# OzAmram/CaloDiffusion

Hardware: AMD Instinct MI355X
Metric: sampled showers/sec (Dataset-2, 400-step DDIM) (higher is better)
Workload: dtype f32 (convs: fp32 operands as 2-term fp16 splits on the fp16 MFMA pipe, fp32 accumulate; attention/norms fp32)

## Files before the change

### calodiffusion_amd/csrc/conv_internal.h

```cpp
#pragma once
#include "kernels_conv.h"
#include "split16.h"
#include <cstdio>
#include <cstdlib>
#include <map>
#include <string>

namespace cd {

#define MFMA32(a, b, c) __builtin_amdgcn_mfma_f32_32x32x2f32((a), (b), (c), 0, 0, 0)
#define MFMA_BF16(a, b, c) __builtin_amdgcn_mfma_f32_32x32x16_bf16(__builtin_bit_cast(bf16x8, (a)), __builtin_bit_cast(bf16x8, (b)), (c), 0, 0, 0)

typedef __bf16 bf16x8 __attribute__((ext_vector_type(8)));
typedef __bf16 bf16x2 __attribute__((ext_vector_type(2)));

__device__ __forceinline__ unsigned pack_bf16(float lo, float hi) {
  const bf16x2 v = {(__bf16)lo, (__bf16)hi};
  return __builtin_bit_cast(unsigned, v);
}
__device__ __forceinline__ void split3(const f32x4 x, u32x2& t1, u32x2& t2, u32x2& t3) {
  f32x4 r = x;
  t1 = u32x2{pack_bf16(r[0], r[1]), pack_bf16(r[2], r[3])};
  r[0] -= __uint_as_float(t1[0] << 16); r[1] -= __uint_as_float(t1[0] & 0xffff0000u);
  r[2] -= __uint_as_float(t1[1] << 16); r[3] -= __uint_as_float(t1[1] & 0xffff0000u);
// ... 39 lines not shown
  int P;
  int cout, CTtot;
  int dbg;
  const float* coef;
  int act;
  float* ch_part;
  int* status = nullptr;
  GnDefer defer;
  int coef_lds_off = 0;
  const unsigned* in_absmax = nullptr;
  const float* add_src = nullptr;
};
bool try_launch_conv3_flat(const float* in0, int c0, const float* in1, int c1, const void* wpk, const float* bias, float* out,
                           int batch, int cout, const ConvGeom& g, hipStream_t s, const ConvFusion& fu,
                           int prec );
bool launch_conv_flat_split16(int VT, int CT, int NTERM, int geo, const ConvFlatArgs& a, dim3 grid, int threads, size_t lds, hipStream_t s);

std::map<std::string, int>& tune_cache();
template <typename F>
int autotune(const std::string& key, int ncand, F&& run, hipStream_t s) {
  auto it = tune_cache().find(key);
  if (it != tune_cache().end()) return it->second;
  hipStreamCaptureStatus st = hipStreamCaptureStatusNone;
  if (getenv("CD_NO_AUTOTUNE") || hipStreamIsCapturing(s, &st) != hipSuccess || st != hipStreamCaptureStatusNone || prof::enabled())
    return -1;
  hipEvent_t e0, e1;
  CD_HIP(hipEventCreate(&e0));
  CD_HIP(hipEventCreate(&e1));
  int best = 0;
  float best_ms = 1e30f;
  for (int i = 0; i < ncand; ++i) {
// ... 20 lines not shown
```

### calodiffusion_amd/csrc/kernels_conv_flat.hip

```cpp
#include "conv_internal.h"
#include "gn_defer.h"
#include <vector>

namespace cd {

template <int VT, int CT>
__global__ void __launch_bounds__(512, (VT * CT <= 2 ? 3 : 2)) conv3_flat_kernel(ConvFlatArgs a) {
  extern __shared__ __attribute__((aligned(16))) float lds[];
  const int tid = threadIdx.x, lane = tid & 63, wave = tid >> 6, nthreads = blockDim.x;
  const int b = blockIdx.y;
  const int ct0 = blockIdx.z * CT;
  const int HW = a.H * a.W;
  const int vox = a.D * HW;
  const int v0 = blockIdx.x * a.R;
  const int vend = min(v0 + a.R, vox);
  const int zA = v0 / HW - 1;
  const int zB = (vend - 1) / HW + 1;
  const int nstage = (zB - zA + 1) * HW;
  const int NZ = a.P * HW;
  const int half = lane >> 5, col = lane & 31;
  if (tid < 16) lds[NZ * 16 + tid] = 0.f;

  int nb[VT], rowm[VT], rowp[VT], ooff[VT];
  unsigned wmask[VT];
// ... 475 lines not shown
  const Dims3 d = g.in;
  const int CTtot = cout / 32;
  const int CTmax = CTtot <= 3 ? CTtot : 2;
  if (CTtot % CTmax) return false;
  const int HW = d.h * d.w, HWo = g.out.h * g.out.w;
  const size_t vox_bytes = prec == 3 ? 96 : (prec == 2 ? 80 : 64);
  auto planes = [&](int NT) { return ((32 * NT - 1) / HWo + 1) * g.sz + g.kd; };
  auto args_for = [&](int NT) {
    ConvFlatArgs a;
    a.in0 = in0; a.in1 = in1; a.c0 = c0; a.c1 = c1; a.wpk = (const float*)wpk; a.bias = bias; a.out = out;
    a.D = d.d; a.H = d.h; a.W = d.w; a.Do = g.out.d; a.Ho = g.out.h; a.Wo = g.out.w;
    a.R = 32 * NT; a.P = planes(NT); a.cout = cout; a.CTtot = CTtot;
    a.coef = fu.coef; a.act = fu.act; a.ch_part = fu.ch_part;
    return a;
  };
  auto launch = [&](int NT, int VT, int CT) -> bool {
    if (VT < 0) {
      const int NLW = -VT;
      ConvFlatArgs a = args_for(NT);
      a.dbg = 0;
      const size_t lds = 2 * ((size_t)a.P * HW + 1) * 96 + (size_t)NT * CT * 64 * 4;
      const int ups = (int)((g.out.vox() + a.R - 1) / a.R);
      const int total = ups * batch;
      const int nblk = total < 256 ? total : 256;
      dim3 grid((unsigned)nblk, 1, (unsigned)(CTtot / CT));
      if (fu.units) *fu.units = ups;
      const int threads = (NT + NLW) * 64;
      switch (CT) {
        case 1: launch_ws_inst<1>(a, grid, threads, lds, NLW, ups, total, s, geo); break;
        case 2: launch_ws_inst<2>(a, grid, threads, lds, NLW, ups, total, s, geo); break;
        case 3: launch_ws_inst<3>(a, grid, threads, lds, NLW, ups, total, s, geo); break;
        default: return false;
      }
      return true;
    }
    ConvFlatArgs a = args_for(NT);
    a.dbg = getenv("CD_FLAT_DBG") ? atoi(getenv("CD_FLAT_DBG")) : 0;
    a.status = fu.status; a.in_absmax = fu.in_absmax;
    a.add_src = prec >= 2 && !bias ? fu.add_src : nullptr;
    size_t lds = ((size_t)a.P * HW + 1) * vox_bytes;
    const size_t red = (size_t)(NT / VT) * CT * 32 * 2 * 4;
    if (lds < red) lds = red;
    if (fu.defer.part) {
      lds = (lds + 15) & ~(size_t)15;
      a.defer = fu.defer;
      a.coef_lds_off = (int)lds;
      lds += (size_t)fu.defer.C * 16 + gn_defer_scratch_bytes(fu.defer.C);
      if (lds > 160 * 1024) return false;
    }
    dim3 grid((unsigned)((g.out.vox() + a.R - 1) / a.R), (unsigned)batch, (unsigned)(CTtot / CT));
    if (fu.units) *fu.units = (int)grid.x;
    const int threads = (NT / VT) * 64;
    const bool launched = prec != 0 ? launch_conv_flat_split16(VT, CT, prec, geo, a, grid, threads, lds, s)
                                    : launch_conv_flat_f32(VT, CT, a, grid, threads, lds, s);
    if (!launched) return false;
    if (a.add_src && fu.add_done) *fu.add_done = 1;
    return true;
  };
  if (const char* ov = getenv("CD_FLAT_TILE")) {
    int nt, vt;
    if (sscanf(ov, "%d,%d", &nt, &vt) == 2 && nt % vt == 0 && nt / vt <= 8 && vt * CTmax <= 8 &&
        ((size_t)planes(nt) * HW + 1) * vox_bytes <= 160 * 1024 && (prec != 2 || vt * CTmax <= 4))
      return launch(nt, vt, CTmax);
  }
  static const int kCand[][2] = {{8, 2}, {4, 1}, {8, 1}, {12, 3}, {16, 2}, {16, 4}, {4, 2}, {6, 2}, {6, 3}, {2, 1},
                                 {3, 1}, {1, 1}, {2, 2}, {12, 2}, {8, 4}, {6, 1}, {3, 3}};
  struct Cand { int nt, vt, ct; };
  std::vector<Cand> cand;
  const bool small = g.out.vox() * batch <= 64 * 1024;
  for (int pass = 0; pass < (small && CTmax > 1 ? 2 : 1); ++pass) {
    const int CT = pass == 0 ? CTmax : 1;
    for (auto& c : kCand) {
      const int NT = c[0], VT = c[1];
      if (VT * CT > 8 || (CT == 3 && VT > 2)) continue;
      if (prec == 2 && VT * CT > 4) continue;
      static const bool no_extra_waves = getenv("CD_FLAT_NO_EXTRA_WAVES") != nullptr;
      const bool extra_ok = !no_extra_waves && g.out.vox() <= 128 && VT == 1 && NT <= 8;
      if ((int64_t)32 * (NT - 1) >= g.out.vox() && !extra_ok) continue;
      if (((size_t)planes(NT) * HW + 1) * vox_bytes > 150 * 1024) continue;
      if (pass == 1 && NT > 4) continue;
      cand.push_back({NT, VT, CT});
    }
  }
  if (prec == 3 && !getenv("CD_NO_WS")) {
    static const int kWs[][2] = {{8, 4}, {8, 2}, {4, 2}, {4, 4}, {8, 3}, {6, 2}, {2, 2}, {3, 1}, {1, 1}, {2, 1}};
    for (auto& c : kWs) {
      const int NMW = c[0], NLW = c[1];
      if ((int64_t)32 * (NMW - 1) >= g.out.vox()) continue;
      const size_t lds = 2 * ((size_t)planes(NMW) * HW + 1) * 96 + (size_t)NMW * CTmax * 64 * 4;
      if (lds > 160 * 1024 - 256) continue;
      cand.push_back({NMW, -NLW, CTmax});
    }
  }
  if (cand.empty()) return false;
  char key[192];
  std::snprintf(key, sizeof key, "flat%s g%d %dx%dx%d c%d+%d->%d b%d", prec == 3 ? "_bf16x3" : (prec == 2 ? "_f16x2" : "_f32"), geo,
                d.d, d.h, d.w, c0, c1, cout, batch);
  const int pick = autotune(key, (int)cand.size(), [&](int i) { launch(cand[i].nt, cand[i].vt, cand[i].ct); }, s);
  const Cand& c = cand[pick < 0 ? 0 : pick];
  return launch(c.nt, c.vt, c.ct);
}

}
```

### calodiffusion_amd/csrc/kernels_conv_flat16.hip

```cpp
#include "conv_internal.h"
#include "gn_defer.h"

namespace cd {

template <int VT, int CT, int KD, int KH, int KW, int SZ, int SXY, int NTERM>
__global__ void __launch_bounds__(512, (VT * CT * (NTERM == 2 ? 2 : 1) <= 2 ? 3 : 2)) conv3_flat_bf16x3_kernel(ConvFlatArgs a) {
  extern __shared__ __attribute__((aligned(16))) float lds[];
  char* ldsb = (char*)lds;
  constexpr int T = KD * KH * KW;
  constexpr int VB = NTERM == 3 ? 96 : 80;
  constexpr int WS = 64 * NTERM;
  const int tid = threadIdx.x, lane = tid & 63, wave = tid >> 6, nthreads = blockDim.x;
  const int b = blockIdx.y;
  const int ct0 = blockIdx.z * CT;
  const int HW = a.H * a.W;
  const int vox = a.D * HW;
  const int HWo = a.Ho * a.Wo;
  const int voxo = a.Do * HWo;
  const int v0 = blockIdx.x * a.R;
  const int vend = min(v0 + a.R, voxo);
  const float inv_hwo = 1.f / (float)HWo, inv_wo = 1.f / (float)a.Wo;
  auto fdiv = [](int x, float inv) { return (int)(((float)x + 0.5f) * inv); };
  const int zA = fdiv(v0, inv_hwo) * SZ - 1;
  const int zB = fdiv(vend - 1, inv_hwo) * SZ + KD - 2;
  const int nstage = (zB - zA + 1) * HW;
  const int NZ = a.P * HW;
  const int half = lane >> 5, col = lane & 31;
  if (a.defer.part) gn_defer_to_lds(a.defer, b, (float*)(ldsb + a.coef_lds_off), ldsb + a.coef_lds_off + a.defer.C * 16);
  const bool normed = a.coef || a.defer.part;
  if (tid < VB / 4) ((float*)(ldsb + (size_t)NZ * VB))[tid] = 0.f;

  int nb[VT], rowoff[VT][KH], ooff[VT];
  unsigned wmask[VT];
  bool any_valid = false;
#pragma unroll
  for (int vt = 0; vt < VT; ++vt) {
    const int v = v0 + (wave * VT + vt) * 32 + col;
    const bool valid = v < vend;
    const int vv = valid ? v : v0;
    const int oz = fdiv(vv, inv_hwo);
    const int r = vv - oz * HWo;
    const int oh = fdiv(r, inv_wo), ow = r - oh * a.Wo;
    const int ih0 = oh * SXY, iw0 = ow * SXY;
    nb[vt] = (oz * SZ - 1 - zA) * HW + ih0 * a.W + iw0;
    unsigned m = 0;
#pragma unroll
    for (int kh = 0; kh < KH; ++kh) {
      int ih = ih0 + kh - 1;
      ih = ih < 0 ? ih + a.H : (ih >= a.H ? ih - a.H : ih);
      ih = ih >= a.H ? ih - a.H : ih;
      rowoff[vt][kh] = (ih - ih0) * a.W;
    }
#pragma unroll
    for (int kw = 0; kw < KW; ++kw) {
      const int iw = iw0 + kw - 1;
      if (valid && iw >= 0 && iw < a.W) m |= 1u << kw;
    }
    wmask[vt] = m;
    ooff[vt] = valid ? v * a.cout : -1;
    any_valid |= valid;
  }
  const bool wave_active = __any(any_valid);

  f32x16 acc[VT][CT], accB[NTERM == 2 ? VT : 1][NTERM == 2 ? CT : 1];
#pragma unroll
  for (int vt = 0; vt < VT; ++vt)
#pragma unroll
    for (int ct = 0; ct < CT; ++ct)
#pragma unroll
      for (int r = 0; r < 16; ++r) {
        acc[vt][ct][r] = 0.f;
        if (NTERM == 2) accB[vt][ct][r] = 0.f;
      }

  float amax = 0.f;
  float gscale = 1.f, ginv = 1.f;
  if (NTERM == 2 && a.in_absmax) pow2_scale_for(*a.in_absmax, &gscale, &ginv);
  const int nsub = (a.c0 + a.c1) >> 4;
  const int gbase = zA * HW;
  const int nslots = nstage * 4;

  auto tap_voxel = [&](int vt, int tap) -> int {
#ifdef CD_FLAT_ABL_TAPS
    return nb[vt] + tap;
#endif
    const int kz = tap / (KH * KW), kh = (tap / KW) % KH, kw = tap % KW;
    const int n = nb[vt] + kz * HW + rowoff[vt][kh] + kw - 1;
    return ((wmask[vt] >> kw) & 1u) ? n : NZ;
  };

  for (int sc = 0; sc < nsub; ++sc) {
    const float* src;
    int ldc, coff;
    if (sc * 16 < a.c0) {
      src = a.in0; ldc = a.c0; coff = sc * 16;
    } else {
      src = a.in1; ldc = a.c1; coff = sc * 16 - a.c0;
    }
    const int pq = tid & 3;
    src += (size_t)b * vox * ldc + coff + pq * 4;
    f32x4 cf[4];
    if (a.defer.part) {
#pragma unroll
      for (int e = 0; e < 4; ++e) cf[e] = *(const f32x4*)(ldsb + a.coef_lds_off + (sc * 16 + pq * 4 + e) * 16);
    } else if (a.coef) {
#pragma unroll
      for (int e = 0; e < 4; ++e) cf[e] = *(const f32x4*)(a.coef + ((size_t)b * (a.c0 + a.c1) + sc * 16 + pq * 4 + e) * 4);
    }
    __syncthreads();
    for (int s0 = tid; s0 < ((a.dbg & 1) ? 0 : nslots); s0 += 4 * nthreads) {
      f32x4 val[4];
#pragma unroll
      for (int k = 0; k < 4; ++k) {
        const int sidx = s0 + k * nthreads;
        const int g = gbase + (sidx >> 2);
        val[k] = f32x4{0.f, 0.f, 0.f, 0.f};
        if (sidx < nslots && g >= 0 && g < vox) {
          val[k] = *(const f32x4*)(src + (size_t)g * ldc);
          if (normed) {
#pragma unroll
            for (int e = 0; e < 4; ++e) {
              float t = cf[e][0] * val[k][e] + cf[e][1];
              if (a.act) t = cd_fast_silu(t);
              val[k][e] = t + cf[e][2];
            }
          }
        }
      }
#pragma unroll
      for (int k = 0; k < 4; ++k) {
        const int sidx = s0 + k * nthreads;
        if (sidx < nslots) {
          char* d = ldsb + (size_t)(sidx >> 2) * VB + pq * 8;
          if (NTERM == 3) {
            u32x2 t1, t2, t3;
            split3(val[k], t1, t2, t3);
            *(u32x2*)d = t1;
            *(u32x2*)(d + 32) = t2;
            *(u32x2*)(d + 64) = t3;
          } else {
            const f32x4 vs = val[k] * gscale;
            amax = fmaxf(amax, fmaxf(fmaxf(fabsf(vs[0]), fabsf(vs[1])), fmaxf(fabsf(vs[2]), fabsf(vs[3]))));
            u32x2 t1, t2;
            split2(vs, t1, t2);
            *(u32x2*)d = t1;
            *(u32x2*)(d + 32) = t2;
          }
        }
      }
    }
    __syncthreads();
    if (!wave_active || (a.dbg & 2)) continue;

#pragma unroll
    for (int vt = 0; vt < VT; ++vt) asm volatile("" : "+v"(nb[vt]));

    const u32x4* wq = (const u32x4*)a.wpk + ((size_t)sc * T * a.CTtot + ct0) * WS + lane;
#ifndef CD_FLAT_WD
#define CD_FLAT_WD 3
#endif
#ifndef CD_FLAT_AD
#define CD_FLAT_AD 2
#endif
    constexpr bool DEEP = NTERM == 2;
    constexpr int WD = DEEP ? CD_FLAT_WD : 1, AD = DEEP ? CD_FLAT_AD : 1;
    u32x4 bw[WD + 1][CT][NTERM], av[AD + 1][VT][NTERM];
    auto load_w = [&](int tap) {
#pragma unroll
      for (int ct = 0; ct < CT; ++ct)
#pragma unroll
        for (int t = 0; t < NTERM; ++t) bw[tap % (WD + 1)][ct][t] = wq[((size_t)tap * a.CTtot + ct) * WS + t * 64];
    };
    auto load_a = [&](int tap) {
#pragma unroll
      for (int vt = 0; vt < VT; ++vt) {
        const char* p = ldsb + (size_t)tap_voxel(vt, tap) * VB + half * 16;
#pragma unroll
        for (int t = 0; t < NTERM; ++t) av[tap % (AD + 1)][vt][t] = *(const u32x4*)(p + t * 32);
      }
    };
#pragma unroll
    for (int t0 = 0; t0 < WD; ++t0) load_w(t0);
#pragma unroll
    for (int t0 = 0; t0 < AD; ++t0) load_a(t0);
#pragma unroll
    for (int tap = 0; tap < T; ++tap) {
      if (tap + WD < T) load_w(tap + WD);
      if (tap + AD < T) load_a(tap + AD);
      __builtin_amdgcn_sched_barrier(0);
      const int wc = tap % (WD + 1), ac = tap % (AD + 1);
#pragma unroll
// ... 6 lines not shown
            c = MFMA_BF16(av[ac][vt][1], bw[wc][ct][1], c);
            c = MFMA_BF16(av[ac][vt][0], bw[wc][ct][NTERM - 1], c);
            c = MFMA_BF16(av[ac][vt][1], bw[wc][ct][0], c);
            c = MFMA_BF16(av[ac][vt][0], bw[wc][ct][1], c);
            c = MFMA_BF16(av[ac][vt][0], bw[wc][ct][0], c);
            acc[vt][ct] = c;
          } else {
            acc[vt][ct] = MFMA_F16(av[ac][vt][0], bw[wc][ct][0], acc[vt][ct]);
            accB[vt][ct] = MFMA_F16(av[ac][vt][0], bw[wc][ct][1], accB[vt][ct]);
            accB[vt][ct] = MFMA_F16(av[ac][vt][1], bw[wc][ct][0], accB[vt][ct]);
          }
        }
    }
  }

  if (NTERM == 2) {
#pragma unroll
    for (int vt = 0; vt < VT; ++vt)
#pragma unroll
      for (int ct = 0; ct < CT; ++ct)
#pragma unroll
        for (int r = 0; r < 16; ++r) acc[vt][ct][r] = (acc[vt][ct][r] + accB[vt][ct][r] * (1.f / 2048.f)) * ginv;
  }
  if (NTERM == 2 && a.status && amax > 65504.f) atomicOr(a.status, 1);
  float* outb = a.out + (size_t)b * voxo * a.cout;
  float bv[CT];
#pragma unroll
  for (int ct = 0; ct < CT; ++ct) bv[ct] = a.bias ? a.bias[(ct0 + ct) * 32 + col] : 0.f;
  if (a.add_src) {
    const float* addb = a.add_src + (size_t)b * voxo * a.cout;
// ... 30 lines not shown
    for (int ct = 0; ct < CT; ++ct) s1[ct] = s2[ct] = 0.f;
#pragma unroll
    for (int vt = 0; vt < VT; ++vt)
#pragma unroll
      for (int r = 0; r < 16; ++r) {
        const int row = (r & 3) + 8 * (r >> 2) + 4 * half;
        const bool ok = __shfl(ooff[vt], row, 64) >= 0;
#pragma unroll
        for (int ct = 0; ct < CT; ++ct) {
          const float v = ok ? acc[vt][ct][r] + bv[ct] : 0.f;
          s1[ct] += v;
          s2[ct] += v * v;
        }
      }
    __syncthreads();
    const int nw = nthreads >> 6;
#pragma unroll
    for (int ct = 0; ct < CT; ++ct) {
      const float t1 = s1[ct] + __shfl_xor(s1[ct], 32, 64), t2 = s2[ct] + __shfl_xor(s2[ct], 32, 64);
      if (half == 0) {
        lds[((wave * CT + ct) * 32 + col) * 2] = t1;
        lds[((wave * CT + ct) * 32 + col) * 2 + 1] = t2;
      }
    }
    __syncthreads();
    for (int i = tid; i < CT * 32; i += nthreads) {
      float t1 = 0.f, t2 = 0.f;
      for (int w = 0; w < nw; ++w) {
        t1 += lds[((w * CT * 32) + i) * 2];
        t2 += lds[((w * CT * 32) + i) * 2 + 1];
      }
      float* dst = a.ch_part + (((size_t)b * gridDim.x + blockIdx.x) * a.cout + ct0 * 32 + i) * 2;
      dst[0] = t1;
      dst[1] = t2;
    }
  }
}

namespace {
template <int VT, int CT, int KD, int KH, int KW, int SZ, int SXY, int NTERM>
void launch_flat3_geo(const ConvFlatArgs& a, dim3 grid, int threads, size_t lds, hipStream_t s) {
  static bool attr_set = false;
  if (!attr_set) {
    CD_HIP(hipFuncSetAttribute((const void*)conv3_flat_bf16x3_kernel<VT, CT, KD, KH, KW, SZ, SXY, NTERM>,
                               hipFuncAttributeMaxDynamicSharedMemorySize, 160 * 1024));
    attr_set = true;
  }
  hipLaunchKernelGGL((conv3_flat_bf16x3_kernel<VT, CT, KD, KH, KW, SZ, SXY, NTERM>), grid, dim3(threads), lds, s, a);
  CD_HIP(hipGetLastError());
}
template <int VT, int CT, int NTERM>
void launch_flat3_inst(const ConvFlatArgs& a, dim3 grid, int threads, size_t lds, hipStream_t s, int geo = 0) {
  if (geo == 0) launch_flat3_geo<VT, CT, 3, 3, 3, 1, 1, NTERM>(a, grid, threads, lds, s);
  else if (geo == 1) launch_flat3_geo<VT, CT, 3, 4, 4, 2, 2, NTERM>(a, grid, threads, lds, s);
  else if (geo == 2) launch_flat3_geo<VT, CT, 3, 4, 4, 1, 2, NTERM>(a, grid, threads, lds, s);
  else launch_flat3_geo<VT, CT, 4, 4, 4, 2, 2, NTERM>(a, grid, threads, lds, s);
}
}

bool launch_conv_flat_split16(int VT, int CT, int NTERM, int geo, const ConvFlatArgs& a, dim3 grid, int threads, size_t lds, hipStream_t s) {
#define CD_FLAT_CASE(V, C)                                                                 \
  if (VT == V && CT == C) {                                                                \
    if (NTERM == 3) launch_flat3_inst<V, C, 3>(a, grid, threads, lds, s, geo);             \
    else if constexpr (V * C <= 4) launch_flat3_inst<V, C, 2>(a, grid, threads, lds, s, geo); \
    else return false;                                                                     \
    return true;                                                                           \
  }
  CD_FLAT_CASE(1, 1) CD_FLAT_CASE(2, 1) CD_FLAT_CASE(3, 1) CD_FLAT_CASE(4, 1)
  CD_FLAT_CASE(1, 2) CD_FLAT_CASE(2, 2) CD_FLAT_CASE(3, 2) CD_FLAT_CASE(4, 2)
  CD_FLAT_CASE(1, 3) CD_FLAT_CASE(2, 3)
#undef CD_FLAT_CASE
  return false;
}

}
```

### calodiffusion_amd/csrc/ops.hip

```cpp
#include "plan_internal.h"

namespace cd {

__global__ void to_cl_kernel(const float* __restrict__ src, float* __restrict__ dst, int channels, int64_t vox) {
  const int b = blockIdx.y;
  const int64_t total = vox * channels;
  for (int64_t i = (int64_t)blockIdx.x * 256 + threadIdx.x; i < total; i += (int64_t)gridDim.x * 256) {
    const int c = (int)(i % channels);
    const int64_t v = i / channels;
    dst[(size_t)b * total + i] = src[(size_t)b * total + (size_t)c * vox + v];
  }
}
__global__ void to_planar_kernel(const float* __restrict__ src, float* __restrict__ dst, int channels, int64_t vox) {
  const int b = blockIdx.y;
  const int64_t total = vox * channels;
  for (int64_t i = (int64_t)blockIdx.x * 256 + threadIdx.x; i < total; i += (int64_t)gridDim.x * 256) {
    const int64_t v = i % vox;
    const int c = (int)(i / vox);
    dst[(size_t)b * total + i] = src[(size_t)b * total + (size_t)v * channels + c];
  }
}
static void launch_transpose_to_cl(const float* ncdhw, float* ndhwc, int batch, int channels, int64_t vox, hipStream_t s) {
  int64_t bx = (vox * channels + 255) / 256;
  if (bx > 1024) bx = 1024;
// ... 66 lines not shown
    CD_REQUIRE(x && w && y && ch_part && units && scratch && chunks >= 0, "bad argument");
    CD_REQUIRE(cin % 32 == 0 && cout % 32 == 0, "channel counts must be multiples of 32");
    hipStream_t s = (hipStream_t)stream;
    launch_pack_weights_f16x2(w, scratch, cout, cin, 27, s);
    const Dims3 d{dims[0], dims[1], dims[2]};
    ConvGeom g{d, d, 3, 3, 3, 1, 1, 1};
    ConvFusion fu;
    int u = 0;
    fu.act = 1; fu.ch_part = ch_part; fu.units = &u; fu.zs_chunks = chunks;
    CD_REQUIRE(try_launch_conv_zslide(x, cin, nullptr, 0, scratch, bias, y, batch, cout, g, s, fu) && u > 0,
               "this grid is not eligible for the z-slide kernel");
    *units = u;
  });
}

int cd_op_cyl_conv_transpose(const float* x, const float* w, const float* bias, float* y, int batch, int channels,
                             const int32_t dims_in[3], int kernel_z, int stride_z, const int32_t out_pad[3],
                             void* scratch, void* stream) {
  return guarded([&] {
    CD_REQUIRE(x && w && y && scratch, "null argument");
    CD_REQUIRE(out_pad[0] == 0, "z output padding is always 0 (models.py:339)");
    hipStream_t s = (hipStream_t)stream;
    float* wpk = (float*)scratch;
    launch_pack_weights(w, wpk, channels, channels, kernel_z * 16, true, s);
    float* wpk16 = wpk + ((packed_weight_floats(channels, channels, kernel_z * 16) + 63) & ~(size_t)63);
    launch_pack_weights_f16x2(w, wpk16, channels, channels, kernel_z * 16, s, true, false);
    const Dims3 din{dims_in[0], dims_in[1], dims_in[2]};
    const Dims3 dout{(din.d - 1) * stride_z - 2 + kernel_z, 2 * din.h + out_pad[1], 2 * din.w + out_pad[2]};
    launch_conv_transpose_mfma(x, channels, wpk, bias, y, batch, channels, din, dout, kernel_z, stride_z, s, wpk16, nullptr);
  });
// ... 173 lines not shown
```

### calodiffusion_amd/engine.py

```python
from __future__ import annotations

import ctypes as C
import os
from typing import Dict, Optional, Sequence

import numpy as np
import torch

_HERE = os.path.dirname(os.path.abspath(__file__))
LIB_PATH = os.environ.get("CALODIFF_LIB") or os.path.join(_HERE, "lib", "libcalodiff_hip.so")

CD_MAX_SIZES = 8
CD_ABI_VERSION = 3
TIME_KINDS = {"log": 0, "sigma": 1, "raw": 2}
OBJECTIVES = {"hybrid": 0, "noise_pred": 1, "mean_pred": 2}
LOSS_TYPES = {"l2": 0, "l1": 1, "mse": 2, "huber": 3}


class CdUnetDesc(C.Structure):
    _fields_ = [
        ("struct_size", C.c_uint32),
        ("grid", C.c_int32 * 3),
        ("in_channels", C.c_int32),
        ("n_sizes", C.c_int32),
# ... 140 lines not shown
                                            C.c_uint64, C.c_uint64, _P, _P, _P, C.c_double, C.c_double, C.c_double, C.c_float, _P, _P,
                                            C.c_size_t, _P]),
    "cd_classifier_dropout_mask": (C.c_int, [C.c_uint64, C.c_uint64, C.c_int, C.c_float, C.c_int, C.c_int, _P, _P]),
    "cd_set_conv_precision": (C.c_int, [C.c_char_p]),
    "cd_get_conv_precision": (C.c_char_p, []),
    "cd_profile_begin": (C.c_int, []),
    "cd_profile_end": (C.c_int, [C.c_char_p, C.c_int]),
    "cd_loss_hybrid_l2": (C.c_int, [_P, C.c_int, _P, _P, _P, _P, _P, _P, C.c_size_t, _P]),
    "cd_loss_hybrid": (C.c_int, [_P, C.c_int, _P, _P, _P, _P, C.c_int, _P, _P, C.c_size_t, _P]),
    "cd_op_to_channels_last": (C.c_int, [_P, _P, C.c_int, C.c_int, C.c_int64, _P]),
    "cd_op_to_ncdhw": (C.c_int, [_P, _P, C.c_int, C.c_int, C.c_int64, _P]),
    "cd_op_cyl_conv": (C.c_int, [_P, C.c_int, _P, C.c_int, _P, _P, _P, C.c_int, C.c_int, C.POINTER(C.c_int32),
                                 C.POINTER(C.c_int32), C.POINTER(C.c_int32), _P, _P]),
    "cd_op_zslide_conv": (C.c_int, [_P, C.c_int, _P, _P, _P, _P, C.POINTER(C.c_int), C.c_int, C.c_int, C.POINTER(C.c_int32), C.c_int,
                                    _P, _P]),
    "cd_op_cyl_conv_transpose": (C.c_int, [_P, _P, _P, _P, C.c_int, C.c_int, C.POINTER(C.c_int32), C.c_int, C.c_int,
                                           C.POINTER(C.c_int32), _P, _P]),
    "cd_op_init_conv": (C.c_int, [_P, _P, _P, _P, C.c_int, C.c_int, C.c_int, C.POINTER(C.c_int32), _P, _P]),
    "cd_op_init_pair_conv": (C.c_int, [_P, _P, _P, _P, _P, C.c_int, _P, _P, _P, C.c_int, C.c_int, _P, _P, _P, C.POINTER(C.c_int), C.c_int,
                                       C.POINTER(C.c_int32), C.c_int, _P, _P]),
    "cd_op_group_norm": (C.c_int, [_P, _P, _P, _P, C.c_int, C.c_int, C.c_int64, C.c_int, C.c_int, _P, _P, _P, _P]),
    "cd_op_resnet_block": (C.c_int, [_P, C.c_int, _P, C.c_int, C.POINTER(_P), _P, _P, C.c_int, C.c_int,
                                     C.POINTER(C.c_int32), C.c_int, _P, C.c_size_t, _P]),
    "cd_op_linear_attention": (C.c_int, [_P, C.POINTER(_P), _P, C.c_int, C.c_int, C.POINTER(C.c_int32), _P, C.c_size_t, _P]),
    "cd_op_conv_backward": (C.c_int, [_P, C.c_int, _P, C.c_int, _P, _P, _P, _P, _P, C.c_int, C.c_int, C.POINTER(C.c_int32),
                                      C.POINTER(C.c_int32), C.POINTER(C.c_int32), _P, C.c_size_t, _P]),
    "cd_op_conv_transpose_backward": (C.c_int, [_P, _P, _P, _P, _P, _P, C.c_int, C.c_int, C.POINTER(C.c_int32), C.c_int, C.c_int,
                                                C.POINTER(C.c_int32), _P, C.c_size_t, _P]),
    "cd_op_group_norm_backward": (C.c_int, [_P, _P, _P, _P, _P, _P, _P, _P, C.c_int, C.c_int, C.c_int64, C.c_int, C.c_int, _P,
                                            C.c_size_t, _P]),
# ... 788 lines not shown

    def zslide_conv_chunked(self, x_cl, w, bias, chunks=0):
        x_cl, w = _dev32(x_cl, "x"), _dev32(w, "w")
        B, D, H, W, cin = x_cl.shape
        cout = w.shape[0]
        y = torch.empty((B, D, H, W, cout), dtype=torch.float32, device=x_cl.device)
        cap = (D * H * W + 31) // 32
        part = torch.zeros((B, cap, cout, 2), dtype=torch.float32, device=x_cl.device)
        units = C.c_int()
        sc = self.scratch(B, max(cin, cout), D * H * W)
        _check(self.lib.cd_op_zslide_conv(x_cl.data_ptr(), cin, w.data_ptr(), _ptr(bias), y.data_ptr(), part.data_ptr(), C.byref(units),
                                          B, cout, _i32x3((D, H, W)), int(chunks), sc.data_ptr(), _stream()))
        u = units.value
        return y, part.view(-1)[:B * u * cout * 2].view(B, u, cout, 2).double().sum(1)

    def cyl_conv_transpose(self, x_cl, w, bias, kernel_z, stride_z, out_pad):
        x_cl, w = _dev32(x_cl, "x"), _dev32(w, "w")
        B, D, H, W, c = x_cl.shape
        od = ((D - 1) * stride_z - 2 + kernel_z, 2 * H + out_pad[1], 2 * W + out_pad[2])
        y = torch.empty((B,) + od + (c,), dtype=torch.float32, device=x_cl.device)
        sc = self.scratch(B, c, int(np.prod(od)))
        _check(self.lib.cd_op_cyl_conv_transpose(x_cl.data_ptr(), w.data_ptr(), _ptr(bias), y.data_ptr(), B, c,
                                                 _i32x3((D, H, W)), kernel_z, stride_z, _i32x3(out_pad), sc.data_ptr(),
                                                 _stream()))
        return y

    def init_conv(self, x_ncdhw, w, bias):
        x, w = _dev32(x_ncdhw, "x"), _dev32(w, "w")
        B, cin, D, H, W = x.shape
        cout = w.shape[0]
# ... 106 lines not shown
```

### include/calodiff.h

```cpp
#ifndef CALODIFF_H
#define CALODIFF_H

#include <stddef.h>
#include <stdint.h>

#ifdef __cplusplus
extern "C" {
#endif

#define CD_OK 0
#define CD_EINVAL -1
#define CD_EHIP -2
#define CD_ENOGPU -3
#define CD_EWEIGHTS -4
#define CD_EWORKSPACE -5

#define CD_MAX_SIZES 8

#define CD_ABI_VERSION 3

#define CD_TIME_LOG 0
#define CD_TIME_SIGMA 1
#define CD_TIME_RAW 2

// ... 261 lines not shown
int cd_classifier_dropout_mask(uint64_t seed, uint64_t step, int layer, float dropout_p, int rows, int n, uint8_t* mask, void* stream);

int cd_set_conv_precision(const char* mode);
const char* cd_get_conv_precision(void);

int cd_profile_begin(void);
int cd_profile_end(char* json, int cap);

int cd_op_to_channels_last(const float* ncdhw, float* ndhwc, int batch, int channels, int64_t voxels, void* stream);
int cd_op_to_ncdhw(const float* ndhwc, float* ncdhw, int batch, int channels, int64_t voxels, void* stream);
int cd_op_cyl_conv(const float* x0, int c0, const float* x1, int c1, const float* w, const float* bias, float* y,
                   int batch, int cout, const int32_t dims_in[3], const int32_t kernel[3], const int32_t stride[3],
                   void* scratch, void* stream);
int cd_op_zslide_conv(const float* x, int cin, const float* w, const float* bias, float* y, float* ch_part, int* units, int batch,
                      int cout, const int32_t dims[3], int chunks, void* scratch, void* stream);
int cd_op_cyl_conv_transpose(const float* x, const float* w, const float* bias, float* y, int batch, int channels,
                             const int32_t dims_in[3], int kernel_z, int stride_z, const int32_t out_pad[3],
                             void* scratch, void* stream);
int cd_op_init_conv(const float* x_ncdhw, const float* w, const float* bias, float* y, int batch, int cin, int cout,
                    const int32_t dims[3], void* scratch, void* stream);
int cd_op_init_pair_conv(const float* x, const float* w0, const float* b0, const float* w1, const float* b1, int cin, const float* r_w,
                         const float* z_d, const float* phi_h, int use_rz, int use_phi, const float* scale_b, float* y, float* ch_part,
                         int* units, int batch, const int32_t dims[3], int slabs, void* scratch, void* stream);
int cd_op_group_norm(const float* x, float* y, const float* gamma, const float* beta, int batch, int channels,
                     int64_t voxels, int groups, int silu, const float* add_bc, const float* residual,
                     void* scratch, void* stream);
int cd_op_resnet_block(const float* x0, int c0, const float* x1, int c1, const float* const* w, const float* cond, float* y,
                       int batch, int cout, const int32_t dims[3], int groups, void* workspace, size_t workspace_bytes,
                       void* stream);
int cd_op_linear_attention(const float* x, const float* const* w, float* y, int batch, int channels, const int32_t dims[3],
// ... 22 lines not shown
```

Measured before the change: 97.17.

## Add flat-conv block forms covering all channel tiles and split-K channel groups

Adds two new launch forms for the f16x2 flat conv kernel. In the first, one block covers every output channel tile, so the staged input image is shared across channel tiles instead of being restaged per grid z-slice. In the second, for small grids, two wave groups each take half the input channel sub-blocks and reduce their partial accumulators through LDS. The change also precomputes per-row LDS tap offsets with edge masks, adds these forms to the autotune candidates, and exposes a test entry point. The cost is larger blocks (up to 1024 threads), extra LDS and extra synchronisation.

```diff
diff --git a/calodiffusion_amd/csrc/conv_internal.h b/calodiffusion_amd/csrc/conv_internal.h
--- a/calodiffusion_amd/csrc/conv_internal.h
+++ b/calodiffusion_amd/csrc/conv_internal.h
@@ -77,7 +77,8 @@
 bool try_launch_conv3_flat(const float* in0, int c0, const float* in1, int c1, const void* wpk, const float* bias, float* out,
                            int batch, int cout, const ConvGeom& g, hipStream_t s, const ConvFusion& fu,
                            int prec );
-bool launch_conv_flat_split16(int VT, int CT, int NTERM, int geo, const ConvFlatArgs& a, dim3 grid, int threads, size_t lds, hipStream_t s);
+bool launch_conv_flat_split16(int VT, int CT, int NTERM, int geo, const ConvFlatArgs& a, dim3 grid, int threads, size_t lds, hipStream_t s,
+                              int form = 0);
 
 std::map<std::string, int>& tune_cache();
 template <typename F>
diff --git a/calodiffusion_amd/csrc/kernels_conv_flat.hip b/calodiffusion_amd/csrc/kernels_conv_flat.hip
--- a/calodiffusion_amd/csrc/kernels_conv_flat.hip
+++ b/calodiffusion_amd/csrc/kernels_conv_flat.hip
@@ -513,7 +513,15 @@
     a.coef = fu.coef; a.act = fu.act; a.ch_part = fu.ch_part;
     return a;
   };
-  auto launch = [&](int NT, int VT, int CT) -> bool {
+  const int nsub = (c0 + c1) / 16;
+  auto form_ok = [&](int NT, int form) {
+    return prec == 2 && geo <= 2 && (form == 1 || (form == 2 && nsub >= 2)) && NT >= 1 && form * CTtot * NT <= 16;
+  };
+  auto lds_image = [&](int NT, int VT, int form) {
+    return (size_t)(prec == 2 && VT == 1 ? g.kw * 80 : 0) + (form == 2 ? 2 : 1) * ((size_t)planes(NT) * HW + 1) * vox_bytes;
+  };
+  auto launch = [&](int NT, int VT, int CT, int form = 0) -> bool {
+    if (form != 0 && !form_ok(NT, form)) return false;
     if (VT < 0) {
       const int NLW = -VT;
       ConvFlatArgs a = args_for(NT);
@@ -537,9 +545,11 @@
     a.dbg = getenv("CD_FLAT_DBG") ? atoi(getenv("CD_FLAT_DBG")) : 0;
     a.status = fu.status; a.in_absmax = fu.in_absmax;
     a.add_src = prec >= 2 && !bias ? fu.add_src : nullptr;
-    size_t lds = ((size_t)a.P * HW + 1) * vox_bytes;
-    const size_t red = (size_t)(NT / VT) * CT * 32 * 2 * 4;
+    size_t lds = lds_image(NT, VT, form);
+    size_t red = (size_t)(NT / VT) * CT * 32 * 2 * 4;
+    if (form != 0) red = (size_t)NT * CTtot * (form == 2 ? 32 * 64 * 4 : 32 * 2 * 4);
     if (lds < red) lds = red;
+    if (lds > 160 * 1024) return false;
     if (fu.defer.part) {
       lds = (lds + 15) & ~(size_t)15;
       a.defer = fu.defer;
@@ -547,24 +557,28 @@
       lds += (size_t)fu.defer.C * 16 + gn_defer_scratch_bytes(fu.defer.C);
       if (lds > 160 * 1024) return false;
     }
-    dim3 grid((unsigned)((g.out.vox() + a.R - 1) / a.R), (unsigned)batch, (unsigned)(CTtot / CT));
-    if (fu.units) *fu.units = (int)grid.x;
-    const int threads = (NT / VT) * 64;
-    const bool launched = prec != 0 ? launch_conv_flat_split16(VT, CT, prec, geo, a, grid, threads, lds, s)
+    dim3 grid((unsigned)((g.out.vox() + a.R - 1) / a.R), (unsigned)batch, (unsigned)(form != 0 ? 1 : CTtot / CT));
+    const int threads = form != 0 ? form * CTtot * NT * 64 : (NT / VT) * 64;
+    const bool launched = prec != 0 ? launch_conv_flat_split16(VT, CT, prec, geo, a, grid, threads, lds, s, form)
                                     : launch_conv_flat_f32(VT, CT, a, grid, threads, lds, s);
     if (!launched) return false;
+    if (fu.units) *fu.units = (int)grid.x;
     if (a.add_src && fu.add_done) *fu.add_done = 1;
     return true;
   };
   if (const char* ov = getenv("CD_FLAT_TILE")) {
-    int nt, vt;
-    if (sscanf(ov, "%d,%d", &nt, &vt) == 2 && nt % vt == 0 && nt / vt <= 8 && vt * CTmax <= 8 &&
-        ((size_t)planes(nt) * HW + 1) * vox_bytes <= 160 * 1024 && (prec != 2 || vt * CTmax <= 4))
+    int nt, vt, form = 0;
+    const int nf = sscanf(ov, "%d,%d,%d", &nt, &vt, &form);
+    if (nf == 3 && form != 0 && prec == 2) {
+      if (vt == 1 && form_ok(nt, form) && launch(nt, 1, 1, form)) return true;
+    } else if (nf >= 2 && nt % vt == 0 && nt / vt <= 8 && vt * CTmax <= 8 &&
+               ((size_t)planes(nt) * HW + 1) * vox_bytes <= 160 * 1024 && (prec != 2 || vt * CTmax <= 4)) {
       return launch(nt, vt, CTmax);
+    }
   }
   static const int kCand[][2] = {{8, 2}, {4, 1}, {8, 1}, {12, 3}, {16, 2}, {16, 4}, {4, 2}, {6, 2}, {6, 3}, {2, 1},
                                  {3, 1}, {1, 1}, {2, 2}, {12, 2}, {8, 4}, {6, 1}, {3, 3}};
-  struct Cand { int nt, vt, ct; };
+  struct Cand { int nt, vt, ct, form; };
   std::vector<Cand> cand;
   const bool small = g.out.vox() * batch <= 64 * 1024;
   for (int pass = 0; pass < (small && CTmax > 1 ? 2 : 1); ++pass) {
@@ -578,7 +592,25 @@
       if ((int64_t)32 * (NT - 1) >= g.out.vox() && !extra_ok) continue;
       if (((size_t)planes(NT) * HW + 1) * vox_bytes > 150 * 1024) continue;
       if (pass == 1 && NT > 4) continue;
-      cand.push_back({NT, VT, CT});
+      cand.push_back({NT, VT, CT, 0});
+    }
+  }
+  if (CTtot >= 2 && geo != 0) {
+    for (int NT : {2, 1, 4}) {
+      if (!form_ok(NT, 1) || NT * CTtot > 8 || (int64_t)32 * (NT - 1) >= g.out.vox() || lds_image(NT, 1, 1) > 150 * 1024) continue;
+      cand.push_back({NT, 1, 1, 1});
+    }
+  }
+  static const int n_simd = [] {
+    int dev = 0, cus = 0;
+    CD_HIP(hipGetDevice(&dev));
+    CD_HIP(hipDeviceGetAttribute(&cus, hipDeviceAttributeMultiprocessorCount, dev));
+    return 4 * cus;
+  }();
+  if ((g.out.vox() + 31) / 32 * batch * CTtot < 2 * (int64_t)n_simd) {
+    for (int NT : {1, 2}) {
+      if (!form_ok(NT, 2) || 2 * NT * CTtot > 8 || (int64_t)32 * (NT - 1) >= g.out.vox() || lds_image(NT, 1, 2) > 150 * 1024) continue;
+      cand.push_back({NT, 1, 1, 2});
     }
   }
   if (prec == 3 && !getenv("CD_NO_WS")) {
@@ -588,16 +620,16 @@
       if ((int64_t)32 * (NMW - 1) >= g.out.vox()) continue;
       const size_t lds = 2 * ((size_t)planes(NMW) * HW + 1) * 96 + (size_t)NMW * CTmax * 64 * 4;
       if (lds > 160 * 1024 - 256) continue;
-      cand.push_back({NMW, -NLW, CTmax});
+      cand.push_back({NMW, -NLW, CTmax, 0});
     }
   }
   if (cand.empty()) return false;
   char key[192];
   std::snprintf(key, sizeof key, "flat%s g%d %dx%dx%d c%d+%d->%d b%d", prec == 3 ? "_bf16x3" : (prec == 2 ? "_f16x2" : "_f32"), geo,
                 d.d, d.h, d.w, c0, c1, cout, batch);
-  const int pick = autotune(key, (int)cand.size(), [&](int i) { launch(cand[i].nt, cand[i].vt, cand[i].ct); }, s);
+  const int pick = autotune(key, (int)cand.size(), [&](int i) { launch(cand[i].nt, cand[i].vt, cand[i].ct, cand[i].form); }, s);
   const Cand& c = cand[pick < 0 ? 0 : pick];
-  return launch(c.nt, c.vt, c.ct);
-}
-
-}
+  return launch(c.nt, c.vt, c.ct, c.form);
+}
+
+}
diff --git a/calodiffusion_amd/csrc/kernels_conv_flat16.hip b/calodiffusion_amd/csrc/kernels_conv_flat16.hip
--- a/calodiffusion_amd/csrc/kernels_conv_flat16.hip
+++ b/calodiffusion_amd/csrc/kernels_conv_flat16.hip
@@ -3,16 +3,29 @@
 
 namespace cd {
 
-template <int VT, int CT, int KD, int KH, int KW, int SZ, int SXY, int NTERM>
-__global__ void __launch_bounds__(512, (VT * CT * (NTERM == 2 ? 2 : 1) <= 2 ? 3 : 2)) conv3_flat_bf16x3_kernel(ConvFlatArgs a) {
+template <int VT, int CT, int KD, int KH, int KW, int SZ, int SXY, int NTERM, int FORM = 0, int MAXT = 512>
+__global__ void __launch_bounds__(MAXT, (MAXT > 512 ? 4 : (VT * CT * (NTERM == 2 ? 2 : 1) <= 2 ? 3 : 2)))
+conv3_flat_bf16x3_kernel(ConvFlatArgs a) {
   extern __shared__ __attribute__((aligned(16))) float lds[];
   char* ldsb = (char*)lds;
   constexpr int T = KD * KH * KW;
   constexpr int VB = NTERM == 3 ? 96 : 80;
   constexpr int WS = 64 * NTERM;
+  constexpr bool PRE = NTERM == 2 && VT == 1;
+  constexpr int IMG = PRE ? KW * VB : 0;
+  constexpr int NG = FORM == 2 ? 2 : 1;
+  static_assert(FORM == 0 || (VT == 1 && CT == 1 && PRE), "forms 1 and 2: one (row tile, channel tile) pair per wave");
   const int tid = threadIdx.x, lane = tid & 63, wave = tid >> 6, nthreads = blockDim.x;
   const int b = blockIdx.y;
-  const int ct0 = blockIdx.z * CT;
+  const int ntile = a.R >> 5;
+  int ct0 = blockIdx.z * CT, tile0 = wave * VT, grp = 0;
+  if (FORM != 0) {
+    const int ws = __builtin_amdgcn_readfirstlane(wave);
+    const int q = (int)(((float)ws + 0.5f) * (1.f / (float)ntile));
+    tile0 = ws - q * ntile;
+    grp = q >= a.CTtot ? 1 : 0;
+    ct0 = q - grp * a.CTtot;
+  }
   const int HW = a.H * a.W;
   const int vox = a.D * HW;
   const int HWo = a.Ho * a.Wo;
@@ -28,14 +41,19 @@
   const int half = lane >> 5, col = lane & 31;
   if (a.defer.part) gn_defer_to_lds(a.defer, b, (float*)(ldsb + a.coef_lds_off), ldsb + a.coef_lds_off + a.defer.C * 16);
   const bool normed = a.coef || a.defer.part;
-  if (tid < VB / 4) ((float*)(ldsb + (size_t)NZ * VB))[tid] = 0.f;
+  const int img_bytes = (NZ + 1) * VB;
+  if (PRE) {
+    for (int i = tid; i < IMG / 4; i += nthreads) ((float*)ldsb)[i] = 0.f;
+  } else if (tid < VB / 4) {
+    ((float*)(ldsb + (size_t)NZ * VB))[tid] = 0.f;
+  }
 
   int nb[VT], rowoff[VT][KH], ooff[VT];
   unsigned wmask[VT];
   bool any_valid = false;
 #pragma unroll
   for (int vt = 0; vt < VT; ++vt) {
-    const int v = v0 + (wave * VT + vt) * 32 + col;
+    const int v = v0 + (tile0 + vt) * 32 + col;
     const bool valid = v < vend;
     const int vv = valid ? v : v0;
     const int oz = fdiv(vv, inv_hwo);
@@ -61,6 +79,16 @@
     any_valid |= valid;
   }
   const bool wave_active = __any(any_valid);
+  unsigned rb[PRE ? KD * KH : 1], mkL = 0, mkR = 0;
+  if constexpr (PRE) {
+#pragma unroll
+    for (int kz = 0; kz < KD; ++kz)
+#pragma unroll
+      for (int kh = 0; kh < KH; ++kh)
+        rb[kz * KH + kh] = (unsigned)(IMG + grp * img_bytes + (nb[0] + kz * HW + rowoff[0][kh] - 1) * VB + half * 16);
+    mkL = (wmask[0] & 1u) ? ~0u : 0u;
+    mkR = ((wmask[0] >> (KW - 1)) & 1u) ? ~0u : 0u;
+  }
 
   f32x16 acc[VT][CT], accB[NTERM == 2 ? VT : 1][NTERM == 2 ? CT : 1];
 #pragma unroll
@@ -89,71 +117,83 @@
     return ((wmask[vt] >> kw) & 1u) ? n : NZ;
   };
 
-  for (int sc = 0; sc < nsub; ++sc) {
-    const float* src;
-    int ldc, coff;
-    if (sc * 16 < a.c0) {
-      src = a.in0; ldc = a.c0; coff = sc * 16;
-    } else {
-      src = a.in1; ldc = a.c1; coff = sc * 16 - a.c0;
-    }
-    const int pq = tid & 3;
-    src += (size_t)b * vox * ldc + coff + pq * 4;
-    f32x4 cf[4];
-    if (a.defer.part) {
-#pragma unroll
-      for (int e = 0; e < 4; ++e) cf[e] = *(const f32x4*)(ldsb + a.coef_lds_off + (sc * 16 + pq * 4 + e) * 16);
-    } else if (a.coef) {
-#pragma unroll
-      for (int e = 0; e < 4; ++e) cf[e] = *(const f32x4*)(a.coef + ((size_t)b * (a.c0 + a.c1) + sc * 16 + pq * 4 + e) * 4);
-    }
-    __syncthreads();
-    for (int s0 = tid; s0 < ((a.dbg & 1) ? 0 : nslots); s0 += 4 * nthreads) {
-      f32x4 val[4];
-#pragma unroll
-      for (int k = 0; k < 4; ++k) {
-        const int sidx = s0 + k * nthreads;
-        const int g = gbase + (sidx >> 2);
-        val[k] = f32x4{0.f, 0.f, 0.f, 0.f};
-        if (sidx < nslots && g >= 0 && g < vox) {
-          val[k] = *(const f32x4*)(src + (size_t)g * ldc);
-          if (normed) {
-#pragma unroll
-            for (int e = 0; e < 4; ++e) {
-              float t = cf[e][0] * val[k][e] + cf[e][1];
-              if (a.act) t = cd_fast_silu(t);
-              val[k][e] = t + cf[e][2];
+  for (int sc0 = 0; sc0 < nsub; sc0 += NG) {
+#pragma unroll
+    for (int j = 0; j < NG; ++j) {
+      const int sc = sc0 + j;
+      if (j > 0 && sc >= nsub) break;
+      const float* src;
+      int ldc, coff;
+      if (sc * 16 < a.c0) {
+        src = a.in0; ldc = a.c0; coff = sc * 16;
+      } else {
+        src = a.in1; ldc = a.c1; coff = sc * 16 - a.c0;
+      }
+      const int pq = tid & 3;
+      src += (size_t)b * vox * ldc + coff + pq * 4;
+      f32x4 cf[4];
+      if (a.defer.part) {
+#pragma unroll
+        for (int e = 0; e < 4; ++e) cf[e] = *(const f32x4*)(ldsb + a.coef_lds_off + (sc * 16 + pq * 4 + e) * 16);
+      } else if (a.coef) {
+#pragma unroll
+        for (int e = 0; e < 4; ++e) cf[e] = *(const f32x4*)(a.coef + ((size_t)b * (a.c0 + a.c1) + sc * 16 + pq * 4 + e) * 4);
+      }
+      if (j == 0) __syncthreads();
+      char* img = ldsb + IMG + j * img_bytes;
+      for (int s0 = tid; s0 < ((a.dbg & 1) ? 0 : nslots); s0 += 4 * nthreads) {
+        f32x4 val[4];
+#pragma unroll
+        for (int k = 0; k < 4; ++k) {
+          const int sidx = s0 + k * nthreads;
+          const int g = gbase + (sidx >> 2);
+          val[k] = f32x4{0.f, 0.f, 0.f, 0.f};
+          if (sidx < nslots && g >= 0 && g < vox) {
+            val[k] = *(const f32x4*)(src + (size_t)g * ldc);
+            if (normed) {
+#pragma unroll
+              for (int e = 0; e < 4; ++e) {
+                float t = cf[e][0] * val[k][e] + cf[e][1];
+                if (a.act) t = cd_fast_silu(t);
+                val[k][e] = t + cf[e][2];
+              }
             }
           }
         }
-      }
-#pragma unroll
-      for (int k = 0; k < 4; ++k) {
-        const int sidx = s0 + k * nthreads;
-        if (sidx < nslots) {
-          char* d = ldsb + (size_t)(sidx >> 2) * VB + pq * 8;
-          if (NTERM == 3) {
-            u32x2 t1, t2, t3;
-            split3(val[k], t1, t2, t3);
-            *(u32x2*)d = t1;
-            *(u32x2*)(d + 32) = t2;
-            *(u32x2*)(d + 64) = t3;
-          } else {
-            const f32x4 vs = val[k] * gscale;
-            amax = fmaxf(amax, fmaxf(fmaxf(fabsf(vs[0]), fabsf(vs[1])), fmaxf(fabsf(vs[2]), fabsf(vs[3]))));
-            u32x2 t1, t2;
-            split2(vs, t1, t2);
-            *(u32x2*)d = t1;
-            *(u32x2*)(d + 32) = t2;
+#pragma unroll
+        for (int k = 0; k < 4; ++k) {
+          const int sidx = s0 + k * nthreads;
+          if (sidx < nslots) {
+            char* d = img + (size_t)(sidx >> 2) * VB + pq * 8;
+            if (NTERM == 3) {
+              u32x2 t1, t2, t3;
+              split3(val[k], t1, t2, t3);
+              *(u32x2*)d = t1;
+              *(u32x2*)(d + 32) = t2;
+              *(u32x2*)(d + 64) = t3;
+            } else {
+              const f32x4 vs = val[k] * gscale;
+              amax = fmaxf(amax, fmaxf(fmaxf(fabsf(vs[0]), fabsf(vs[1])), fmaxf(fabsf(vs[2]), fabsf(vs[3]))));
+              u32x2 t1, t2;
+              split2(vs, t1, t2);
+              *(u32x2*)d = t1;
+              *(u32x2*)(d + 32) = t2;
+            }
           }
         }
       }
     }
     __syncthreads();
-    if (!wave_active || (a.dbg & 2)) continue;
-
-#pragma unroll
-    for (int vt = 0; vt < VT; ++vt) asm volatile("" : "+v"(nb[vt]));
+    const int sc = sc0 + grp;
+    if (!wave_active || (a.dbg & 2) || (NG > 1 && sc >= nsub)) continue;
+
+    if constexpr (!PRE) {
+#pragma unroll
+      for (int vt = 0; vt < VT; ++vt) asm volatile("" : "+v"(nb[vt]));
+    } else {
+#pragma unroll
+      for (int i = 0; i < KD * KH; ++i) asm volatile("" : "+v"(rb[i]));
+    }
 
     const u32x4* wq = (const u32x4*)a.wpk + ((size_t)sc * T * a.CTtot + ct0) * WS + lane;
 #ifndef CD_FLAT_WD
@@ -174,7 +214,16 @@
     auto load_a = [&](int tap) {
 #pragma unroll
       for (int vt = 0; vt < VT; ++vt) {
-        const char* p = ldsb + (size_t)tap_voxel(vt, tap) * VB + half * 16;
+        const char* p;
+        if constexpr (PRE) {
+          const int kz = tap / (KH * KW), kh = (tap / KW) % KH, kw = tap % KW;
+          unsigned o = rb[kz * KH + kh];
+          if (kw == 0) o &= mkL;
+          else if (kw == KW - 1) o &= mkR;
+          p = ldsb + o + kw * VB;
+        } else {
+          p = ldsb + (size_t)tap_voxel(vt, tap) * VB + half * 16;
+        }
 #pragma unroll
         for (int t = 0; t < NTERM; ++t) av[tap % (AD + 1)][vt][t] = *(const u32x4*)(p + t * 32);
       }
@@ -211,6 +260,26 @@
     }
   }
 
+  if constexpr (FORM == 2) {
+    __syncthreads();
+    float* xch = (float*)ldsb + (size_t)(ct0 * ntile + tile0) * 32 * 64 + lane;
+    if (grp == 1) {
+#pragma unroll
+      for (int r = 0; r < 16; ++r) {
+        xch[r * 64] = acc[0][0][r];
+        xch[(16 + r) * 64] = accB[0][0][r];
+      }
+      ooff[0] = -1;
+    }
+    __syncthreads();
+    if (grp == 0) {
+#pragma unroll
+      for (int r = 0; r < 16; ++r) {
+        acc[0][0][r] += xch[r * 64];
+        accB[0][0][r] += xch[(16 + r) * 64];
+      }
+    }
+  }
   if (NTERM == 2) {
 #pragma unroll
     for (int vt = 0; vt < VT; ++vt)
@@ -271,6 +340,26 @@
         }
       }
     __syncthreads();
+    if constexpr (FORM != 0) {
+      const float t1 = s1[0] + __shfl_xor(s1[0], 32, 64), t2 = s2[0] + __shfl_xor(s2[0], 32, 64);
+      if (half == 0 && grp == 0) {
+        lds[((ct0 * ntile + tile0) * 32 + col) * 2] = t1;
+        lds[((ct0 * ntile + tile0) * 32 + col) * 2 + 1] = t2;
+      }
+      __syncthreads();
+      for (int i = tid; i < a.CTtot * 32; i += nthreads) {
+        const int base = ((i >> 5) * ntile * 32 + (i & 31)) * 2;
+        float t1 = 0.f, t2 = 0.f;
+        for (int w = 0; w < ntile; ++w) {
+          t1 += lds[base + w * 64];
+          t2 += lds[base + w * 64 + 1];
+        }
+        float* dst = a.ch_part + (((size_t)b * gridDim.x + blockIdx.x) * a.cout + i) * 2;
+        dst[0] = t1;
+        dst[1] = t2;
+      }
+      return;
+    }
     const int nw = nthreads >> 6;
 #pragma unroll
     for (int ct = 0; ct < CT; ++ct) {
@@ -295,16 +384,24 @@
 }
 
 namespace {
-template <int VT, int CT, int KD, int KH, int KW, int SZ, int SXY, int NTERM>
+template <int VT, int CT, int KD, int KH, int KW, int SZ, int SXY, int NTERM, int FORM = 0, int MAXT = 512>
 void launch_flat3_geo(const ConvFlatArgs& a, dim3 grid, int threads, size_t lds, hipStream_t s) {
   static bool attr_set = false;
   if (!attr_set) {
-    CD_HIP(hipFuncSetAttribute((const void*)conv3_flat_bf16x3_kernel<VT, CT, KD, KH, KW, SZ, SXY, NTERM>,
+    CD_HIP(hipFuncSetAttribute((const void*)conv3_flat_bf16x3_kernel<VT, CT, KD, KH, KW, SZ, SXY, NTERM, FORM, MAXT>,
                                hipFuncAttributeMaxDynamicSharedMemorySize, 160 * 1024));
     attr_set = true;
   }
-  hipLaunchKernelGGL((conv3_flat_bf16x3_kernel<VT, CT, KD, KH, KW, SZ, SXY, NTERM>), grid, dim3(threads), lds, s, a);
+  hipLaunchKernelGGL((conv3_flat_bf16x3_kernel<VT, CT, KD, KH, KW, SZ, SXY, NTERM, FORM, MAXT>), grid, dim3(threads), lds, s, a);
   CD_HIP(hipGetLastError());
+}
+template <int FORM, int MAXT>
+bool launch_flat3_form(const ConvFlatArgs& a, dim3 grid, int threads, size_t lds, hipStream_t s, int geo) {
+  if (geo == 0) launch_flat3_geo<1, 1, 3, 3, 3, 1, 1, 2, FORM, MAXT>(a, grid, threads, lds, s);
+  else if (geo == 1) launch_flat3_geo<1, 1, 3, 4, 4, 2, 2, 2, FORM, MAXT>(a, grid, threads, lds, s);
+  else if (geo == 2) launch_flat3_geo<1, 1, 3, 4, 4, 1, 2, 2, FORM, MAXT>(a, grid, threads, lds, s);
+  else return false;
+  return true;
 }
 template <int VT, int CT, int NTERM>
 void launch_flat3_inst(const ConvFlatArgs& a, dim3 grid, int threads, size_t lds, hipStream_t s, int geo = 0) {
@@ -315,8 +412,15 @@
 }
 }
 
-bool launch_conv_flat_split16(int VT, int CT, int NTERM, int geo, const ConvFlatArgs& a, dim3 grid, int threads, size_t lds, hipStream_t s) {
-#define CD_FLAT_CASE(V, C)                                                                 \
+bool launch_conv_flat_split16(int VT, int CT, int NTERM, int geo, const ConvFlatArgs& a, dim3 grid, int threads, size_t lds, hipStream_t s,
+                              int form) {
+  if (form != 0) {
+    if (NTERM != 2 || VT != 1 || CT != 1 || threads > 1024) return false;
+    if (form == 1) return threads > 512 ? launch_flat3_form<1, 1024>(a, grid, threads, lds, s, geo) : launch_flat3_form<1, 512>(a, grid, threads, lds, s, geo);
+    if (form == 2) return threads > 512 ? launch_flat3_form<2, 1024>(a, grid, threads, lds, s, geo) : launch_flat3_form<2, 512>(a, grid, threads, lds, s, geo);
+    return false;
+  }
+#define CD_FLAT_CASE(V, C)                                                                \
   if (VT == V && CT == C) {                                                                \
     if (NTERM == 3) launch_flat3_inst<V, C, 3>(a, grid, threads, lds, s, geo);             \
     else if constexpr (V * C <= 4) launch_flat3_inst<V, C, 2>(a, grid, threads, lds, s, geo); \
diff --git a/calodiffusion_amd/csrc/ops.hip b/calodiffusion_amd/csrc/ops.hip
--- a/calodiffusion_amd/csrc/ops.hip
+++ b/calodiffusion_amd/csrc/ops.hip
@@ -1,4 +1,5 @@
 #include "plan_internal.h"
+#include "conv_internal.h"
 
 namespace cd {
 
@@ -104,6 +105,47 @@
   });
 }
 
+int cd_op_flat_conv(const float* x0, int c0, const float* x1, int c1, const float* w, const float* bias, float* y, int batch, int cout,
+                    const int32_t dims_in[3], const int32_t kernel[3], const int32_t stride[3], const float* gn_part, int gn_units,
+                    const float* gn_gamma, const float* gn_beta, const float* gn_add, int gn_groups, int act, int rescale,
+                    const float* add_src, float* ch_part, int* units, int* status, void* scratch, void* stream) {
+  return guarded([&] {
+    CD_REQUIRE(x0 && w && y && units && status && scratch, "null argument");
+    CD_REQUIRE(c0 > 0 && c0 % 16 == 0 && c1 % 16 == 0 && cout % 32 == 0, "input channels in multiples of 16, output channels of 32");
+    CD_REQUIRE(!gn_part || (c1 == 0 && gn_gamma && gn_beta && gn_units > 0 && gn_groups > 0), "bad normalisation arguments");
+    CD_REQUIRE(!(rescale || add_src) || (!bias && !(rescale && gn_part)), "rescaling and the added tensor need bias == null");
+    hipStream_t s = (hipStream_t)stream;
+    const int taps = kernel[0] * kernel[1] * kernel[2], cin = c0 + c1;
+    char* w3 = (char*)scratch;
+    launch_pack_weights_split16(w, (float*)w3, cout, cin, taps, s);
+    unsigned* words = (unsigned*)(w3 + ((packed_split16_bytes(cin, cout, taps) + 255) & ~(size_t)255));
+    CD_HIP(hipMemsetAsync(words, 0, sizeof(unsigned) * 4, s));
+    const Dims3 din{dims_in[0], dims_in[1], dims_in[2]};
+    ConvGeom g;
+    g.in = din;
+    g.kd = kernel[0]; g.kh = kernel[1]; g.kw = kernel[2]; g.sz = stride[0]; g.sh = stride[1]; g.sw = stride[2];
+    g.out = Dims3{(din.d + 2 - g.kd) / g.sz + 1, (din.h + 2 - g.kh) / g.sh + 1, (din.w + 2 - g.kw) / g.sw + 1};
+    ConvFusion fu;
+    int u = 0, added = 0;
+    fu.act = act; fu.ch_part = ch_part; fu.units = &u; fu.status = (int*)words; fu.add_src = add_src; fu.add_done = &added;
+    if (gn_part) {
+      fu.defer.part = gn_part; fu.defer.units = gn_units; fu.defer.gamma = gn_gamma; fu.defer.beta = gn_beta; fu.defer.add = gn_add;
+      fu.defer.add_ld = cin; fu.defer.C = cin; fu.defer.groups = gn_groups; fu.defer.vox = din.vox();
+    }
+    if (rescale) {
+      AbsmaxWords aw{words + 1, words + 4};
+      CD_REQUIRE(c1 == 0, "rescaling measures a single source");
+      fu.in_absmax = launch_absmax_bits(x0, (size_t)batch * din.vox() * c0, &aw, s);
+    }
+    CD_REQUIRE(try_launch_conv3_flat(x0, c0, x1, c1, w3 + packed_bf16x3_bytes(cin, cout, taps), bias, y, batch, cout, g, s, fu, 2),
+               "this conv is not eligible for the f16x2 flat-range kernel");
+    CD_REQUIRE(!add_src || added, "internal: the flat kernel did not add the tensor");
+    *units = u;
+    CD_HIP(hipMemcpyAsync(status, words, sizeof(int), hipMemcpyDeviceToHost, s));
+    CD_HIP(hipStreamSynchronize(s));
+  });
+}
+
 int cd_op_cyl_conv_transpose(const float* x, const float* w, const float* bias, float* y, int batch, int channels,
                              const int32_t dims_in[3], int kernel_z, int stride_z, const int32_t out_pad[3],
                              void* scratch, void* stream) {
diff --git a/calodiffusion_amd/engine.py b/calodiffusion_amd/engine.py
--- a/calodiffusion_amd/engine.py
+++ b/calodiffusion_amd/engine.py
@@ -178,6 +178,9 @@
                                  C.POINTER(C.c_int32), C.POINTER(C.c_int32), _P, _P]),
     "cd_op_zslide_conv": (C.c_int, [_P, C.c_int, _P, _P, _P, _P, C.POINTER(C.c_int), C.c_int, C.c_int, C.POINTER(C.c_int32), C.c_int,
                                     _P, _P]),
+    "cd_op_flat_conv": (C.c_int, [_P, C.c_int, _P, C.c_int, _P, _P, _P, C.c_int, C.c_int, C.POINTER(C.c_int32), C.POINTER(C.c_int32),
+                                  C.POINTER(C.c_int32), _P, C.c_int, _P, _P, _P, C.c_int, C.c_int, C.c_int, _P, _P, C.POINTER(C.c_int),
+                                  C.POINTER(C.c_int), _P, _P]),
     "cd_op_cyl_conv_transpose": (C.c_int, [_P, _P, _P, _P, C.c_int, C.c_int, C.POINTER(C.c_int32), C.c_int, C.c_int,
                                            C.POINTER(C.c_int32), _P, _P]),
     "cd_op_init_conv": (C.c_int, [_P, _P, _P, _P, C.c_int, C.c_int, C.c_int, C.POINTER(C.c_int32), _P, _P]),
@@ -996,6 +999,27 @@
         u = units.value
         return y, part.view(-1)[:B * u * cout * 2].view(B, u, cout, 2).double().sum(1)
 
+    def flat_conv(self, x_cl, w, bias=None, stride=(1, 1, 1), x1_cl=None, gn=None, rescale=False, add_src=None):
+        x_cl, w = _dev32(x_cl, "x"), _dev32(w, "w")
+        B, D, H, W, c0 = x_cl.shape
+        c1 = 0 if x1_cl is None else x1_cl.shape[-1]
+        cout, k = w.shape[0], tuple(w.shape[2:])
+        od = ((D + 2 - k[0]) // stride[0] + 1, (H + 2 - k[1]) // stride[1] + 1, (W + 2 - k[2]) // stride[2] + 1)
+        y = torch.empty((B,) + od + (cout,), dtype=torch.float32, device=x_cl.device)
+        cap = (od[0] * od[1] * od[2] + 31) // 32
+        part = torch.zeros((B, cap, cout, 2), dtype=torch.float32, device=x_cl.device)
+        units, status = C.c_int(), C.c_int()
+        sc = self.scratch(B, max(c0 + c1, cout), D * H * W)
+        g = gn or {}
+        gpart = g.get("part")
+        _check(self.lib.cd_op_flat_conv(x_cl.data_ptr(), c0, _ptr(x1_cl), c1, w.data_ptr(), _ptr(bias), y.data_ptr(), B, cout,
+                                        _i32x3((D, H, W)), _i32x3(k), _i32x3(stride), _ptr(gpart), 0 if gpart is None else gpart.shape[1],
+                                        _ptr(g.get("gamma")), _ptr(g.get("beta")), _ptr(g.get("add")), int(g.get("groups", 0)),
+                                        int(g.get("act", 0)), int(bool(rescale)), _ptr(add_src), part.data_ptr(), C.byref(units),
+                                        C.byref(status), sc.data_ptr(), _stream()))
+        u = units.value
+        return y, part.view(-1)[:B * u * cout * 2].view(B, u, cout, 2).clone(), status.value
+
     def cyl_conv_transpose(self, x_cl, w, bias, kernel_z, stride_z, out_pad):
         x_cl, w = _dev32(x_cl, "x"), _dev32(w, "w")
         B, D, H, W, c = x_cl.shape
diff --git a/include/calodiff.h b/include/calodiff.h
--- a/include/calodiff.h
+++ b/include/calodiff.h
@@ -299,6 +299,10 @@
                    void* scratch, void* stream);
 int cd_op_zslide_conv(const float* x, int cin, const float* w, const float* bias, float* y, float* ch_part, int* units, int batch,
                       int cout, const int32_t dims[3], int chunks, void* scratch, void* stream);
+int cd_op_flat_conv(const float* x0, int c0, const float* x1, int c1, const float* w, const float* bias, float* y, int batch, int cout,
+                    const int32_t dims_in[3], const int32_t kernel[3], const int32_t stride[3], const float* gn_part, int gn_units,
+                    const float* gn_gamma, const float* gn_beta, const float* gn_add, int gn_groups, int act, int rescale,
+                    const float* add_src, float* ch_part, int* units, int* status, void* scratch, void* stream);
 int cd_op_cyl_conv_transpose(const float* x, const float* w, const float* bias, float* y, int batch, int channels,
                              const int32_t dims_in[3], int kernel_z, int stride_z, const int32_t out_pad[3],
                              void* scratch, void* stream);
```

Measured after the change: 98.01, median of 6. Within noise of the previous version (+0.9%).
